# microsoft/Spartan2

Measured on AMD Instinct MI355X. Metric: sha256_spartan prove(): R1CS constraints/sec (prove wall-clock in ms_per_step), higher is better.
Workload: dtype u256 modular integer (8 x u32 Montgomery limbs; T256 scalar/base fields)

## Files before the change

### spartan2_amd/csrc/capi_core.hip

```cpp
#include <atomic>
#include <chrono>
#include <cstdlib>
#include <cstdio>
#include <cstring>

#include "core.hpp"
#include "walk_pool.hpp"
#include "kernels_poly.hpp"
#include "sumcheck_round.hpp"

namespace sp {
static thread_local std::string g_err;
static thread_local sp_wait_hook g_wait_hook = nullptr;
static thread_local void* g_wait_user = nullptr;
void set_error(const std::string& m) { g_err = m; }
static std::atomic<int> g_live_contexts{0};
int live_contexts() { return g_live_contexts.load(std::memory_order_relaxed); }
void relax() {
  if (g_wait_hook) g_wait_hook(g_wait_user);
  else __builtin_ia32_pause();
}
void slow_note(const char* site, long spins) {
  static const bool on = getenv("SPARTAN_SLOWPATH_LOG") != nullptr;
  if (on) fprintf(stderr, "[slow path] %s after %ld polls\n", site, spins);
// ... 1487 lines not shown
      }
      return 1;
    }
    if (round + 1 >= rounds) {
      if (ahead) return 0;
      sp_table* tabs[2] = {A, B};
      have_sums = false;
      int rc2 = launch_bind(c, tabs, 2, rv);
      return rc2 ? rc2 : 1;
    }
    const bool gated = ahead && !launch_ahead_ok(c, A->len);
    if (gated && !gate_ok(c)) return 0;
    if (!stopped && tail_enabled() && A->len <= TAIL_MAX_LEN && table_dense(A) && table_dense(B) && lease.take(tail_blocks(A->len / 2))) {
      spk::TailArgs ta;
      ta.A = A->d;
      ta.B = B->d;
      ta.C = nullptr;
      ta.len = A->len;
      ta.r0 = rv;
      ta.eq_pl = ta.eq_pr = nullptr;
      ta.ell = ta.first_half = ta.rnd0 = 0;
      ta.mail = c->d_mail;
      ta.mirror = c->d_mail_mirror;
      ta.r0_from_mail = ahead ? 1 : 0;
      ta.mapped = c->d_pinned;
      ta.seq0 = next_seq(c);
      ta.hand_n = tail_hand_n(false);
      tail_nb0 = tail_blocks(A->len / 2);
      hipLaunchKernelGGL((spk::k_sumcheck_tail<false>), dim3(tail_nb0), dim3(spk::TAIL_THREADS), 0, c->stream, ta);
      if (!c->tail_ev) (void)hipEventCreateWithFlags(&c->tail_ev, hipEventDisableTiming);
      if (c->tail_ev && hipEventRecord(c->tail_ev, c->stream) == hipSuccess) c->tail_ev_pending = true;
      in_tail = true;
      have_sums = true;
      sp::after_bind(A);
      sp::after_bind(B);
      c->pending_slots = tail_blocks(A->len);
      return 1;
    }
    const bool dense = table_dense(A) && table_dense(B);
    const bool sparse_stream = !dense && A->len / 4 >= STREAM_MIN_Q && sp::eff_lo(A) == A->len / 2 && sp::eff_lo(B) == B->len / 2 && sp::eff_hi(A) <= A->len / 4 && sp::eff_hi(B) <= B->len / 4;
    if (gated && !dense && !sparse_stream) return 0;
    const spk::MailRef mref = gated ? gate_launch(c, answers) : mail_ref(c, ahead, answers);
    if (dense) {
      const size_t q = A->len / 4;
      size_t blocks = (q + chunk - 1) / chunk;
      if (q >= STREAM_MIN_Q) {
        const unsigned seq = next_seq(c);
        const spk::LazyOut lp = lazy_out(c, reinterpret_cast<spk::lazy9_t*>(c->d_scratch), q / 256, 2, nullptr, seq);
        c->timed("bind_stream_quad", 48ull * A->len * 2, [&] {
          hipLaunchKernelGGL(spk::k_bind_eval_quad_stream, dim3((unsigned)(q / 256)), dim3(256), 0, c->stream, A->d, B->d, q, rv, lp, mref);
        });
        sum_lazy_launch(c, lp, q / 256);
      } else {
        c->timed("bind", 48ull * A->len * 2, [&] {
          hipLaunchKernelGGL(spk::k_bind_eval_quad, dim3((unsigned)blocks), dim3(256), 0, c->stream, A->d, B->d, q, rv, c->d_scratch, c->d_pinned, next_seq(c), mref);
        });
        reduce_partials_launch(c, blocks, 2);
      }
      sp::after_bind(A);
      sp::after_bind(B);
      have_sums = true;
      return 1;
    }
    if (sparse_stream) {
      const size_t q = A->len / 4;
      const unsigned seq = next_seq(c);
      const spk::LazyOut lp = lazy_out(c, reinterpret_cast<spk::lazy9_t*>(c->d_scratch), q / 256, 2, nullptr, seq);
      c->timed("bind_stream_quad_sparse", 64ull * (A->len / 2) * 2, [&] {
        hipLaunchKernelGGL(spk::k_bind_eval_quad_stream_sparse, dim3((unsigned)(q / 256)), dim3(256), 0, c->stream, A->d, B->d, q, rv, sp::eff_hi(A), sp::eff_hi(B), lp,
                           mref);
      });
      sum_lazy_launch(c, lp, q / 256);
      sp::after_bind(A);
      sp::after_bind(B);
      have_sums = true;
      return 1;
    }
    if (ahead) return 0;
    sp_table* tabs[2] = {A, B};
    have_sums = false;
    int rc2 = launch_bind(c, tabs, 2, rv);
    return rc2 ? rc2 : 1;
  };
  for (size_t round = 0; round < rounds; ++round) {
    const size_t half = A->len / 2, len_now = A->len;
    const double tr0 = round_trace() ? now_us() : 0;
    fe_t sums[2] = {fe_zero(), fe_zero()};
    bool waiting = have_sums;
    if (!have_sums && !host_mode) {
      size_t len = sp::eff_pairs(A);
      if (sp::eff_pairs(B) < len) len = sp::eff_pairs(B);
      if (half < len) len = half;
      if (len >= STREAM_MIN_Q && len % 1024 == 0) {
        const unsigned seq = next_seq(c);
        const size_t hi_max = sp::eff_hi(A) > sp::eff_hi(B) ? sp::eff_hi(A) : sp::eff_hi(B);
        const bool lowhi = hi_max <= len / 2;
        const size_t blocks = len / (256 * (size_t)4);
        const spk::LazyOut lp = lazy_out(c, reinterpret_cast<spk::lazy9_t*>(c->d_scratch), blocks, 2, nullptr, seq);
        c->timed("eval_quad", 64ull * len + 32ull * ((sp::eff_hi(A) < len ? sp::eff_hi(A) : len) + (sp::eff_hi(B) < len ? sp::eff_hi(B) : len)), [&] {
          if (lowhi)
            hipLaunchKernelGGL((spk::k_eval_quad_stream_lowhi<4>), dim3((unsigned)blocks), dim3(256), 0, c->stream, A->d, B->d, half, sp::eff_hi(A), sp::eff_hi(B), lp);
          else
            hipLaunchKernelGGL((spk::k_eval_quad_stream<4>), dim3((unsigned)blocks), dim3(256), 0, c->stream, A->d, B->d, half, sp::eff_hi(A), sp::eff_hi(B), lp);
        });
        sum_lazy_launch(c, lp, blocks);
        waiting = true;
      } else if (len > 0) {
        size_t blocks = (len + chunk - 1) / chunk;
        c->timed("eval_quad", 64ull * len + 32ull * ((sp::eff_hi(A) < len ? sp::eff_hi(A) : len) + (sp::eff_hi(B) < len ? sp::eff_hi(B) : len)),
                 [&] { hipLaunchKernelGGL(spk::k_eval_quad, dim3((unsigned)blocks), dim3(256), 0, c->stream, A->d, B->d, half, len, sp::eff_hi(A), sp::eff_hi(B), c->d_scratch, c->d_pinned, next_seq(c)); });
        reduce_partials_launch(c, blocks, 2);
        waiting = true;
      }
    }
    const unsigned wait_seq = c->result_seq, wait_slots = c->pending_slots;
    const bool wait_resident = in_tail;
    if (wait_resident && !host_mode && spk::tail_hand_over(len_now, tail_hand_n(false))) {
      hA.resize(2 * len_now);
      if ((rc = wait_hand_over(c, wait_seq, (int)(2 * len_now), hA.data()))) return rc;
      hB = hA.data() + len_now;
      host_mode = true;
      hand_seq = wait_seq;
    }
    if (host_mode) {
      host_quad_eval(hA.data(), hB, half, sums);
      waiting = false;
    }
    if (!host_mode && wait_resident && spk::tail_double(false, len_now, tail_hand_n(false))) {
      fe_t S8[8];
      if ((rc = wait_wide(c, wait_seq, spk::TAIL_DOUBLE_SUMS_QUAD, S8))) return rc;
      if (reduce) {
        int hrc = reduce(reduce_user, reinterpret_cast<uint64_t*>(S8), 8);
        if (hrc) return fail(hrc, "prove_quad: the reduce hook failed");
      }
      fe_t rr[2];
      for (int half2 = 0; half2 < 2; ++half2) {
        fe_t e0, tinf;
        if (half2 == 0) {
          e0 = fe_add<S>(S8[0], S8[1]);
          tinf = fe_add<S>(S8[2], S8[3]);
        } else {
          const fe_t r = rr[0];
          e0 = fe_add<S>(S8[0], fe_mul<S>(r, fe_add<S>(fe_sub<S>(fe_sub<S>(S8[4], S8[0]), S8[2]), fe_mul<S>(r, S8[2]))));
          tinf = fe_add<S>(S8[5], fe_mul<S>(r, fe_add<S>(fe_sub<S>(fe_sub<S>(S8[7], S8[5]), S8[6]), fe_mul<S>(r, S8[6]))));
        }
        UniPoly poly;
        poly.n = 3;
        poly.c[0] = e0;
        poly.c[1] = fe_sub<S>(fe_sub<S>(claim, fe_dbl<S>(e0)), tinf);
        poly.c[2] = tinf;
        absorb_poly(tr->t, poly);
        if (!tr->t.squeeze<S>(lbl_c, 1, &rr[half2])) return fail(SP_ERR_INTERNAL_TRANSCRIPT, "transcript round counter overflow");
        tail_post_challenge(c, rr[half2], wait_seq + half2);
        store_fe(out_r + 4 * (round + half2), rr[half2]);
        store_fe(out_cpolys + 8 * (round + half2), poly.c[0]);
        store_fe(out_cpolys + 8 * (round + half2) + 4, poly.c[2]);
        claim = poly_eval(poly, rr[half2]);
      }
      for (int k = 0; k < 2; ++k) {
        sp::after_bind(A);
        sp::after_bind(B);
        next_seq(c);
      }
      have_sums = round + 2 < rounds;
      c->pending_slots = have_sums ? 1u : 0u;
      last_answered = wait_seq + 1;
      guard.armed = round + 2 < rounds;
      if (observe)
        for (int k = 0; k < 2; ++k) {
          uint64_t rw[4];
          store_fe(rw, rr[k]);
          observe(observe_user, round + k, rw);
        }
      if (round_trace()) fprintf(stderr, "quad rounds %2zu+%2zu len %8zu tail 2 wait+host %7.1f us\n", round, round + 1, len_now, now_us() - tr0);
      ++round;
      continue;
    }
    int issued = 0;
    if (!host_mode && waiting && (in_tail || (c->mail_dev && !reduce))) {
      issued = issue(round, nullptr, wait_seq);
      if (issued < 0) return issued;
      guard.armed = issued != 0;
    }
    if (waiting) {
      const unsigned cur_seq = c->result_seq, cur_slots = c->pending_slots;
      c->result_seq = wait_seq;
      c->pending_slots = wait_slots;
      rc = reduce_partials_wait(c, 2, sums, wait_resident || issued != 0);
      if (issued) {
        c->result_seq = cur_seq;
        c->pending_slots = cur_slots;
      }
      if (rc) return rc;
    }
    if (reduce) {
      int hrc = reduce(reduce_user, reinterpret_cast<uint64_t*>(sums), 2);
      if (hrc) return fail(hrc, "prove_quad: the reduce hook failed");
    }
    const double tr1 = round_trace() ? now_us() : 0;
    fe_t e0 = sums[0], tinf = sums[1];
    UniPoly poly;
    poly.n = 3;
    poly.c[0] = e0;
    poly.c[1] = fe_sub<S>(fe_sub<S>(claim, fe_dbl<S>(e0)), tinf);
    poly.c[2] = tinf;
    absorb_poly(tr->t, poly);
    fe_t r_i;
    if (!tr->t.squeeze<S>(lbl_c, 1, &r_i)) return fail(SP_ERR_INTERNAL_TRANSCRIPT, "transcript round counter overflow");
    last_answered = wait_seq;
    if (host_mode) {
      host_bind_tables(hA.data(), (size_t)(hB - hA.data()), 2, len_now, r_i);
      sp::after_bind(A);
      sp::after_bind(B);
      have_sums = false;
    } else if (issued) {
      tail_post_challenge(c, r_i, wait_seq);
    } else {
      issued = issue(round, &r_i, wait_seq);
      if (issued < 0) return issued;
      if (wait_resident) tail_post_challenge(c, r_i, wait_seq);
    }
    store_fe(out_r + 4 * round, r_i);
    store_fe(out_cpolys + 8 * round, poly.c[0]);
    store_fe(out_cpolys + 8 * round + 4, poly.c[2]);
    claim = poly_eval(poly, r_i);
    guard.armed = in_tail && (host_mode || round + 1 < rounds);
    if (observe) {
      uint64_t rw[4];
      store_fe(rw, r_i);
      observe(observe_user, round, rw);
    }
    if (round_trace()) fprintf(stderr, "quad round %2zu len %8zu tail %d wait %7.1f us host %6.1f us\n", round, len_now, (int)wait_resident, tr1 - tr0, now_us() - tr1);
  }
  if (stopped) {
    store_fe(claim_io, claim);
    return tail_check(c);
  }
  if (host_mode) {
    store_fe(out_final, hA[0]);
    store_fe(out_final + 4, hB[0]);
    tail_post_challenge(c, hA[0], hand_seq);
// ... 1092 lines not shown
```

### spartan2_amd/csrc/kernels_poly.hpp

```cpp
#pragma once
#include "device_utils.hpp"
#include "kernels_shared.hpp"

namespace spk {

constexpr int RESULT_FLAG_ELEM = 7;
__device__ __forceinline__ void publish_result(fe_t* result, unsigned seq) {
  __threadfence_system();
  __hip_atomic_store(reinterpret_cast<unsigned*>(result + RESULT_FLAG_ELEM), seq, __ATOMIC_RELEASE, __HIP_MEMORY_SCOPE_SYSTEM);
}

template <int NACC>
__device__ __forceinline__ void emit_partials_wide(const fe_t (&acc)[NACC], fe_t* __restrict__ mapped, unsigned seq);
template <int NACC>
__device__ __forceinline__ void emit_partials(const fe_t (&acc)[NACC], fe_t* __restrict__ partials, fe_t* __restrict__ mapped, unsigned seq) {
  if (gridDim.x <= HOST_SUM_MAX_BLOCKS) {
    fe_t* slot = mapped + SLOT_BASE_ELEM + 4 * blockIdx.x;
    slot_chk chk = {0u, 0u};
#pragma unroll
    for (int k = 0; k < NACC; ++k) {
      slot_store_elem(slot + k, acc[k]);
      slot_chk_add(chk, acc[k], k);
    }
    slot_store_tag(slot, seq, chk);
// ... 79 lines not shown
    const unsigned* line = mail + MAIL_LINE_WORDS * (want & (MAIL_RING - 1));
    const unsigned* mline = mirror ? mirror + MAIL_LINE_WORDS * (want & (MAIL_RING - 1)) : nullptr;
    const unsigned long long t0 = wall_clock64();
    unsigned long long next_mirror = t0 + MAIL_MIRROR_AFTER_TICKS;
    int good = 0, aborted = 0, from_mirror = 0;
    unsigned w = 0, wdev = 0;
    for (unsigned it = 0;; ++it) {
      if (lane < 13) w = __hip_atomic_load(line + lane, __ATOMIC_RELAXED, __HIP_MEMORY_SCOPE_SYSTEM);
      int st = 0;
      if (__builtin_amdgcn_readlane((int)w, 12) != 0 || ((unsigned)__builtin_amdgcn_readlane((int)w, 8) == want && (unsigned)__builtin_amdgcn_readlane((int)w, 11) == want))
        st = mail_line_state(w, want, lane);
      const bool tick = (it & 15u) == 15u;
      if (st == 0 && mline && tick) {
        const unsigned long long now = wall_clock64();
        if (now >= next_mirror) {
          wdev = w;
          unsigned wm = 0;
          if (lane < 13) wm = __hip_atomic_load(mline + lane, __ATOMIC_RELAXED, __HIP_MEMORY_SCOPE_SYSTEM);
          st = mail_line_state(wm, want, lane);
          if (st != 0) {
            w = wm;
            from_mirror = 1;
          }
          next_mirror = now + MAIL_MIRROR_EVERY_TICKS;
        }
      }
      if (st < 0) {
        aborted = 1;
        break;
      }
      if (st > 0) {
        good = 1;
        break;
      }
      if (tick && wall_clock64() - t0 > MAIL_WATCHDOG_TICKS) break;
    }
    if (lane < 8) r_smem->v[lane] = w;
    if (mline && lane == 0 && (from_mirror || (!good && !aborted))) {
      unsigned* diag = const_cast<unsigned*>(mail) + MAIL_DIAG_WORD;
      if (from_mirror) {
        atomicAdd(diag + 0, 1u);
        diag[2] = want;
      } else {
        atomicAdd(diag + 1, 1u);
      }
    }
    if (mline && from_mirror && lane == 8) const_cast<unsigned*>(mail)[MAIL_DIAG_WORD + 3] = wdev;
    if (!good && !aborted) {
      const unsigned seen = lane < 13 ? w : 0u;
      if (lane < 13) reinterpret_cast<unsigned*>(mapped + TAIL_ERR_ELEM + 1)[lane] = seen;
      if (lane == 0) {
        unsigned* e = reinterpret_cast<unsigned*>(mapped + TAIL_ERR_ELEM);
        e[1] = want;
        e[2] = blockIdx.x;
        e[3] = gridDim.x;
        __hip_atomic_store(e, 1u, __ATOMIC_RELEASE, __HIP_MEMORY_SCOPE_SYSTEM);
      }
    }
    if (lane == 0) ok = good;
  }
  __syncthreads();
  return ok != 0;
}
__device__ __forceinline__ fe_t gated_challenge(const fe_t* p) {
  typedef const __attribute__((address_space(4))) uint32_t* const_words;
  const_words q = (const_words)(uintptr_t)p;
  fe_t r;
#pragma unroll
  for (int i = 0; i < 8; ++i) r.v[i] = q[i];
  return r;
}
__device__ __forceinline__ fe_t challenge_or(const MailRef& m, const fe_t& r_arg) {
  if (m.gated) return gated_challenge(m.gated);
  if (!m.mail) return r_arg;
  __shared__ fe_t r_sh;
  mail_wait(m.mail, m.mirror, m.mapped, m.answers, &r_sh);
  return r_sh;
}

__global__ void __launch_bounds__(64) k_mail_gate(MailRef m, fe_t* __restrict__ out) {
  __shared__ fe_t r_sh;
  mail_wait(m.mail, m.mirror, m.mapped, m.answers, &r_sh);
  if (threadIdx.x < 8) out->v[threadIdx.x] = r_sh.v[threadIdx.x];
}

constexpr int BIND_MAX_TABLES = 8;
struct BindArgs {
  fe_t* z[BIND_MAX_TABLES];
  unsigned long long n[BIND_MAX_TABLES];
  unsigned long long lo[BIND_MAX_TABLES];
  unsigned long long hi[BIND_MAX_TABLES];
  fe_t r;
  fe_t one_minus_r;
};
__global__ void __launch_bounds__(256) k_bind_top(BindArgs a) {
  const int t = blockIdx.y;
  fe_t* __restrict__ Z = a.z[t];
  const unsigned long long n = a.n[t], lo = a.lo[t], hi = a.hi[t];
  const unsigned long long eff = lo > hi ? lo : hi;
  const unsigned long long both = lo < hi ? lo : hi;
  for (unsigned long long i = (unsigned long long)blockIdx.x * blockDim.x + threadIdx.x; i < eff; i += (unsigned long long)gridDim.x * blockDim.x) {
    fe_t out;
    if (i < both) {
      fe_t lo_v = Z[i], hi_v = Z[n + i];
      out = fe_add<S>(lo_v, fe_mul<S>(a.r, fe_sub<S>(hi_v, lo_v)));
    } else if (i < lo) {
      out = fe_mul<S>(Z[i], a.one_minus_r);
    } else {
      out = fe_mul<S>(a.r, Z[n + i]);
    }
    Z[i] = out;
  }
}

__global__ void __launch_bounds__(1024) k_eq_levels(const fe_t* __restrict__ v, int m, fe_t* __restrict__ out) {
  __shared__ fe_t lv[EQ_LDS_ENTRIES];
  eq_levels_block(v + (m - 1), m, out, lv);
}
struct EqPairArgs {
  fe_t v[2][16];
  int m[2];
  fe_t* out[2];
};
__global__ void __launch_bounds__(1024) k_eq_levels_pair(EqPairArgs a) {
  __shared__ fe_t lv[EQ_LDS_ENTRIES];
  const int b = blockIdx.x;
  const int m = a.m[b];
  eq_levels_block(&a.v[b][m - 1], m, a.out[b], lv);
}
constexpr int EQ_LASTK_HPB = 8;
constexpr int EQ_LASTK_BLOCK = 512;
struct EqLastK {
  fe_t w[16];
};
__global__ void __launch_bounds__(EQ_LASTK_BLOCK) k_eq_outer_lastk(const fe_t* __restrict__ t_hi, const fe_t* __restrict__ t_lo, int K, size_t n_hi, EqLastK wk,
                                                                   fe_t* __restrict__ out) {
  constexpr unsigned SLICES = 1024 / EQ_LASTK_BLOCK;
  const unsigned t = threadIdx.x + (blockIdx.x % SLICES) * EQ_LASTK_BLOCK;
  const size_t hi0 = (size_t)(blockIdx.x / SLICES) * EQ_LASTK_HPB;
  fe_t th[EQ_LASTK_HPB];
#pragma unroll
  for (int h = 0; h < EQ_LASTK_HPB; ++h) th[h] = t_hi[hi0 + h < n_hi ? hi0 + h : 0];
  const fe_t lo = fe_mul<S>(t_lo[t >> K], wk.w[t & ((1u << K) - 1)]);
#pragma unroll
  for (int h = 0; h < EQ_LASTK_HPB; ++h) {
    if (hi0 + h >= n_hi) break;
    out[((hi0 + h) << 10) + t] = fe_mul<S>(th[h], lo);
  }
}
__global__ void __launch_bounds__(256) k_eq_outer(const fe_t* __restrict__ t_hi, const fe_t* __restrict__ t_lo, int lo_bits, size_t total,
                                                  fe_t* __restrict__ out) {
  const size_t mask = ((size_t)1 << lo_bits) - 1;
  for (size_t i = (size_t)blockIdx.x * blockDim.x + threadIdx.x; i < total; i += (size_t)gridDim.x * blockDim.x)
    out[i] = fe_mul<S>(t_hi[i >> lo_bits], t_lo[i & mask]);
}

constexpr int EVAL_PPT = 1;
template <int MODE, bool WITH_M1, bool ZC = false>
__global__ void __launch_bounds__(256) k_eval_cubic(const fe_t* __restrict__ A, const fe_t* __restrict__ B, const fe_t* __restrict__ C, size_t half,
                                                    const fe_t* __restrict__ eq_in, const fe_t* __restrict__ eq_out, int s,
                                                    fe_t* __restrict__ partials, fe_t* __restrict__ single_out, unsigned seq) {
  constexpr int NACC = WITH_M1 ? 3 : 2;
  __shared__ fe_t smem[NACC * 4];
  const size_t chunk = (size_t)blockDim.x * EVAL_PPT;
  const size_t base = (size_t)blockIdx.x * chunk;
  const size_t mask = ((size_t)1 << s) - 1;
// ... 243 lines not shown
  bool nz = false;
#pragma unroll
  for (int k = 0; k < PPT; ++k) nz |= !fe_is_zero(p0[k]);
  lazy9_t l0 = lazy_from(fe_zero()), l1 = lazy_from(fe_zero());
#pragma unroll
  for (int k = 0; k < PPT; ++k) l1 = lazy_add(l1, lazy_from(fe_mul<S>(w[k], p1[k])));
  l1 = lazy_wave_sum(l1);
  if (__any(nz)) {
#pragma unroll
    for (int k = 0; k < PPT; ++k) l0 = lazy_add(l0, lazy_from(fe_mul<S>(w[k], p0[k])));
    l0 = lazy_wave_sum(l0);
  }
  stream_block_partials(l0, l1, partials);
}
__global__ void __launch_bounds__(256) k_bind_eval_quad_stream(fe_t* __restrict__ A, fe_t* __restrict__ B, size_t q, fe_t r_arg, LazyOut partials,
                                                               MailRef mref) {
  const size_t id = (size_t)blockIdx.x * blockDim.x + threadIdx.x;
  const fe_t la0 = A[id], la1 = A[id + q], la2 = A[id + 2 * q], la3 = A[id + 3 * q];
  const fe_t lb0 = B[id], lb1 = B[id + q], lb2 = B[id + 2 * q], lb3 = B[id + 3 * q];
  const fe_t r = challenge_or(mref, r_arg);
  const fe_t a0 = bind1(la0, la2, r), a1 = bind1(la1, la3, r);
  const fe_t b0 = bind1(lb0, lb2, r), b1 = bind1(lb1, lb3, r);
  A[id] = a0;
  A[id + q] = a1;
  B[id] = b0;
  B[id + q] = b1;
  stream_block_partials(lazy_wave_sum(lazy_from(fe_mul<S>(a0, b0))), lazy_wave_sum(lazy_from(fe_mul<S>(fe_sub<S>(a1, a0), fe_sub<S>(b1, b0)))), partials);
}
__global__ void __launch_bounds__(256) k_bind_eval_quad_stream_sparse(fe_t* __restrict__ A, fe_t* __restrict__ B, size_t q, fe_t r_arg, size_t hiA, size_t hiB,
                                                                      LazyOut partials, MailRef mref) {
  const size_t id = (size_t)blockIdx.x * blockDim.x + threadIdx.x;
  const fe_t la0 = A[id], la1 = A[id + q], lb0 = B[id], lb1 = B[id + q];
  const fe_t r = challenge_or(mref, r_arg);
  const fe_t one_minus_r = fe_sub<S>(fe_one<S>(), r);
  const fe_t a0 = id < hiA ? bind1(la0, A[id + 2 * q], r) : fe_mul<S>(la0, one_minus_r);
  const fe_t b0 = id < hiB ? bind1(lb0, B[id + 2 * q], r) : fe_mul<S>(lb0, one_minus_r);
  const fe_t a1 = fe_mul<S>(la1, one_minus_r), b1 = fe_mul<S>(lb1, one_minus_r);
  A[id] = a0;
  A[id + q] = a1;
  B[id] = b0;
  B[id + q] = b1;
  stream_block_partials(lazy_wave_sum(lazy_from(fe_mul<S>(a0, b0))), lazy_wave_sum(lazy_from(fe_mul<S>(fe_sub<S>(a1, a0), fe_sub<S>(b1, b0)))), partials);
}
template <int PPT>
__global__ void __launch_bounds__(256) k_eval_quad_stream(const fe_t* __restrict__ A, const fe_t* __restrict__ B, size_t half, size_t hiA, size_t hiB,
                                                          LazyOut partials) {
  const size_t stride = (size_t)gridDim.x * blockDim.x;
  size_t id = (size_t)blockIdx.x * blockDim.x + threadIdx.x;
  lazy9_t l0 = lazy_from(fe_zero()), l1 = lazy_from(fe_zero());
#pragma unroll
  for (int k = 0; k < PPT; ++k, id += stride) {
    const fe_t a0 = A[id], b0 = B[id];
    const fe_t a1 = id < hiA ? A[id + half] : fe_zero(), b1 = id < hiB ? B[id + half] : fe_zero();
    l0 = lazy_add(l0, lazy_from(fe_mul<S>(a0, b0)));
    l1 = lazy_add(l1, lazy_from(fe_mul<S>(fe_sub<S>(a1, a0), fe_sub<S>(b1, b0))));
  }
  stream_block_partials(lazy_wave_sum(l0), lazy_wave_sum(l1), partials);
}
template <int PPT>
__global__ void __launch_bounds__(256) k_eval_quad_stream_lowhi(const fe_t* __restrict__ A, const fe_t* __restrict__ B, size_t half, size_t hiA, size_t hiB,
                                                                LazyOut partials) {
  const size_t stride = (size_t)gridDim.x * blockDim.x;
  const size_t id0 = (size_t)blockIdx.x * blockDim.x + threadIdx.x;
  fe_t a0[PPT], b0[PPT];
#pragma unroll
  for (int k = 0; k < PPT; ++k) {
    a0[k] = A[id0 + k * stride];
    b0[k] = B[id0 + k * stride];
  }
  lazy9_t l0 = lazy_from(fe_zero()), l1 = lazy_from(fe_zero());
#pragma unroll
  for (int k = 0; k < PPT; ++k) {
    const size_t id = id0 + k * stride;
    const fe_t p = fe_mul<S>(a0[k], b0[k]);
    l0 = lazy_add(l0, lazy_from(p));
    if (id < hiA || id < hiB) {
      const fe_t a1 = id < hiA ? A[id + half] : fe_zero(), b1 = id < hiB ? B[id + half] : fe_zero();
      l1 = lazy_add(l1, lazy_from(fe_sub<S>(fe_mul<S>(fe_sub<S>(a1, a0[k]), fe_sub<S>(b1, b0[k])), p)));
    }
  }
  l1 = lazy_add(l1, l0);
  stream_block_partials(lazy_wave_sum(l0), lazy_wave_sum(l1), partials);
}
template <int GL>
__global__ void __launch_bounds__(64) k_sum_partials_lazy(const uint32_t* __restrict__ P, size_t nparts, int gl_rt, const fe_t* __restrict__ eq_out,
                                                          fe_t* __restrict__ mapped, unsigned seq) {
  const int gl = GL >= 0 ? GL : gl_rt;
  const size_t ngroups = nparts >> gl, per = (size_t)1 << gl;
  fe_t acc[2] = {fe_zero(), fe_zero()};
  for (size_t g = (size_t)blockIdx.x * 64 + threadIdx.x; g < ngroups; g += (size_t)gridDim.x * 64) {
    unsigned long long col[2][9];
#pragma unroll
    for (int w = 0; w < 9; ++w)
#pragma unroll
      for (int a = 0; a < 2; ++a) {
        const uint32_t* src = P + (size_t)(2 * w + a) * nparts + g * per;
        if constexpr (GL == 0) {
          col[a][w] = src[0];
        } else if constexpr (GL == 1) {
          const uint2 v = *reinterpret_cast<const uint2*>(src);
          col[a][w] = (unsigned long long)v.x + v.y;
        } else if constexpr (GL == 2) {
          const uint4 v = *reinterpret_cast<const uint4*>(src);
          col[a][w] = ((unsigned long long)v.x + v.y) + ((unsigned long long)v.z + v.w);
        } else if constexpr (GL == 3) {
          const uint4 v = *reinterpret_cast<const uint4*>(src), u = *reinterpret_cast<const uint4*>(src + 4);
          col[a][w] = (((unsigned long long)v.x + v.y) + ((unsigned long long)v.z + v.w)) + (((unsigned long long)u.x + u.y) + ((unsigned long long)u.z + u.w));
        } else {
          unsigned long long t = 0;
          for (size_t k = 0; k < per; ++k) t += src[k];
          col[a][w] = t;
        }
      }
    fe_t f[2];
#pragma unroll
    for (int a = 0; a < 2; ++a) {
      lazy9_t l;
      unsigned long long carry = 0;
#pragma unroll
      for (int w = 0; w < 9; ++w) {
        const unsigned long long t = col[a][w] + carry;
        l.v[w] = (uint32_t)t;
        carry = t >> 32;
      }
      f[a] = lazy_reduce(l);
    }
    if (eq_out) {
      const fe_t eo = eq_out[g];
      f[0] = fe_mul<S>(f[0], eo);
      f[1] = fe_mul<S>(f[1], eo);
    }
    acc[0] = fe_add<S>(acc[0], f[0]);
    acc[1] = fe_add<S>(acc[1], f[1]);
  }
  acc[0] = wave_sum(acc[0]);
  acc[1] = wave_sum(acc[1]);
  if (threadIdx.x == 0) emit_partials<2>(acc, nullptr, mapped, seq);
}

__global__ void __launch_bounds__(256) k_eval_quad(const fe_t* __restrict__ A, const fe_t* __restrict__ B, size_t half, size_t len, size_t hiA, size_t hiB,
                                                   fe_t* __restrict__ partials, fe_t* __restrict__ single_out, unsigned seq) {
  __shared__ fe_t smem[2 * 4];
  const size_t chunk = (size_t)blockDim.x * EVAL_PPT;
  const size_t base = (size_t)blockIdx.x * chunk;
  fe_t acc[2] = {fe_zero(), fe_zero()};
#pragma unroll 1
  for (int k = 0; k < EVAL_PPT; ++k) {
    const size_t id = base + (size_t)k * blockDim.x + threadIdx.x;
    if (id < len) {
      const fe_t a0 = A[id], b0 = B[id];
      const fe_t a1 = id < hiA ? A[id + half] : fe_zero(), b1 = id < hiB ? B[id + half] : fe_zero();
      acc[0] = fe_add<S>(acc[0], fe_mul<S>(a0, b0));
      acc[1] = fe_add<S>(acc[1], fe_mul<S>(fe_sub<S>(a1, a0), fe_sub<S>(b1, b0)));
    }
  }
  block_sum<2>(acc, smem);
  if (threadIdx.x == 0) {
    emit_partials<2>(acc, partials, single_out, seq);
  }
}

template <bool FALLBACK>
__global__ void __launch_bounds__(256) k_eval_cubic_outer_pow(const fe_t* __restrict__ pleft, size_t left, const fe_t* __restrict__ pright, size_t right,
                                                              const fe_t* __restrict__ A, const fe_t* __restrict__ B, const fe_t* __restrict__ C, size_t len,
                                                              fe_t* __restrict__ partials, fe_t* __restrict__ single_out, unsigned seq) {
  __shared__ fe_t smem[3 * 4];
  fe_t acc[3] = {fe_zero(), fe_zero(), fe_zero()};
  const size_t low = (size_t)blockIdx.x * blockDim.x + threadIdx.x;
  if (low < len) {
    fe_t tl, th;
    if (FALLBACK) {
      tl = pleft[low];
      th = pleft[low + len];
    } else {
      const size_t i = low % left, j = low / left;
      const fe_t pl = pleft[i];
      tl = fe_mul<S>(pl, pright[j]);
      th = fe_mul<S>(pl, pright[j + right]);
    }
    const fe_t al = A[low], ah = A[low + len], bl = B[low], bh = B[low + len], cl = C[low], ch = C[low + len];
    acc[0] = fe_mul<S>(tl, fe_sub<S>(fe_mul<S>(al, bl), cl));
    fe_t tb = fe_sub<S>(fe_dbl<S>(th), tl), ab = fe_sub<S>(fe_dbl<S>(ah), al), bb = fe_sub<S>(fe_dbl<S>(bh), bl), cb = fe_sub<S>(fe_dbl<S>(ch), cl);
    acc[1] = fe_mul<S>(tb, fe_sub<S>(fe_mul<S>(ab, bb), cb));
    tb = fe_sub<S>(fe_add<S>(tb, th), tl);
    ab = fe_sub<S>(fe_add<S>(ab, ah), al);
    bb = fe_sub<S>(fe_add<S>(bb, bh), bl);
    cb = fe_sub<S>(fe_add<S>(cb, ch), cl);
    acc[2] = fe_mul<S>(tb, fe_sub<S>(fe_mul<S>(ab, bb), cb));
  }
  block_sum<3>(acc, smem);
  if (threadIdx.x == 0) {
    emit_partials<3>(acc, partials, single_out, seq);
  }
}

struct CubicPairArgs {
  const fe_t *A[2], *B[2], *C[2];
};
template <bool FALLBACK>
__global__ void __launch_bounds__(256) k_eval_cubic_outer_pow_pair(const fe_t* __restrict__ pleft, size_t left, const fe_t* __restrict__ pright, size_t right,
                                                                   CubicPairArgs t, size_t len, unsigned nb, unsigned pp, fe_t* __restrict__ mapped, unsigned seq) {
  __shared__ fe_t smem[3 * 4];
  const unsigned inst = blockIdx.x / nb, bx = blockIdx.x % nb;
  const fe_t* __restrict__ A = t.A[inst];
  const fe_t* __restrict__ B = t.B[inst];
  const fe_t* __restrict__ C = t.C[inst];
  fe_t acc[3] = {fe_zero(), fe_zero(), fe_zero()};
  for (unsigned k = 0; k < pp; ++k) {
    const size_t low = ((size_t)bx * pp + k) * blockDim.x + threadIdx.x;
    if (low >= len) break;
    fe_t tl, th;
    if (FALLBACK) {
      tl = pleft[low];
      th = pleft[low + len];
    } else {
      const size_t i = low % left, j = low / left;
      const fe_t pl = pleft[i];
      tl = fe_mul<S>(pl, pright[j]);
      th = fe_mul<S>(pl, pright[j + right]);
    }
// ... 526 lines not shown
```

Before: 1.024 billion.

## Fuse first two quad sumcheck rounds into one eval and one double-bind pass

Adds a fast path for the first two rounds of the quadratic sumcheck when the high halves of both tables are a short live prefix. One streaming kernel computes the partial sums both rounds need from the quarter tables, plus a small prefix correction. A fused kernel then binds both challenges in one pass, gated on the mailbox so it can be queued ahead. The aim is to avoid one full read/write pass over the tables and one host round trip, at the cost of more complex gating and sums-assembly logic.

After: 1.060 billion (median of 6 runs). +3.5%, better.

```diff
diff --git a/spartan2_amd/csrc/capi_core.hip b/spartan2_amd/csrc/capi_core.hip
--- a/spartan2_amd/csrc/capi_core.hip
+++ b/spartan2_amd/csrc/capi_core.hip
@@ -1593,7 +1593,108 @@
     int rc2 = launch_bind(c, tabs, 2, rv);
     return rc2 ? rc2 : 1;
   };
+  auto two_rounds = [&](const fe_t S8[8], size_t round, unsigned wait_seq, bool post, fe_t rr[2]) -> int {
+    for (int half2 = 0; half2 < 2; ++half2) {
+      fe_t e0, tinf;
+      if (half2 == 0) {
+        e0 = fe_add<S>(S8[0], S8[1]);
+        tinf = fe_add<S>(S8[2], S8[3]);
+      } else {
+        const fe_t r = rr[0];
+        e0 = fe_add<S>(S8[0], fe_mul<S>(r, fe_add<S>(fe_sub<S>(fe_sub<S>(S8[4], S8[0]), S8[2]), fe_mul<S>(r, S8[2]))));
+        tinf = fe_add<S>(S8[5], fe_mul<S>(r, fe_add<S>(fe_sub<S>(fe_sub<S>(S8[7], S8[5]), S8[6]), fe_mul<S>(r, S8[6]))));
+      }
+      UniPoly poly;
+      poly.n = 3;
+      poly.c[0] = e0;
+      poly.c[1] = fe_sub<S>(fe_sub<S>(claim, fe_dbl<S>(e0)), tinf);
+      poly.c[2] = tinf;
+      absorb_poly(tr->t, poly);
+      if (!tr->t.squeeze<S>(lbl_c, 1, &rr[half2])) return fail(SP_ERR_INTERNAL_TRANSCRIPT, "transcript round counter overflow");
+      if (post) tail_post_challenge(c, rr[half2], wait_seq + half2);
+      store_fe(out_r + 4 * (round + half2), rr[half2]);
+      store_fe(out_cpolys + 8 * (round + half2), poly.c[0]);
+      store_fe(out_cpolys + 8 * (round + half2) + 4, poly.c[2]);
+      claim = poly_eval(poly, rr[half2]);
+    }
+    return SP_OK;
+  };
+  static_assert(spk::QUAD2_HI_MAX <= STREAM_MIN_Q, "the two-round kernels take a live prefix of the high halves that lies inside the third quarter");
+  const bool first_two = !reduce && rounds >= 2 && A->len >= 4 * STREAM_MIN_Q && sp::eff_lo(A) == A->len / 2 && sp::eff_lo(B) == B->len / 2 &&
+                         sp::eff_hi(A) <= spk::QUAD2_HI_MAX && sp::eff_hi(B) <= spk::QUAD2_HI_MAX;
+  auto first_two_rounds = [&]() -> int {
+    const double tr0 = round_trace() ? now_us() : 0;
+    const size_t len = A->len, q = len / 4, e = len / 8, hiA = sp::eff_hi(A), hiB = sp::eff_hi(B), hi = hiA > hiB ? hiA : hiB;
+    const unsigned nprefix = (unsigned)((hi + 255) / 256), nparts = (unsigned)(q / 512);
+    spk::lazy9_t* P = reinterpret_cast<spk::lazy9_t*>(c->d_scratch);
+    const unsigned seq = next_seq(c);
+    c->timed("eval_quad", 32ull * len + 128ull * hi + 32ull * (hiA + hiB), [&] {
+      hipLaunchKernelGGL((spk::k_eval_quad2_stream_lowhi<2>), dim3(nprefix + nparts), dim3(256), 0, c->stream, A->d, B->d, q, hiA, hiB, nprefix, P, c->d_pinned, seq);
+    });
+    const unsigned nslots = (unsigned)((nparts / 4 + 63) / 64);
+    hipLaunchKernelGGL((spk::k_sum_partials_lazy<2, 3>), dim3(nslots), dim3(64), 0, c->stream, reinterpret_cast<const uint32_t*>(P), (size_t)nparts, 2,
+                       (const fe_t*)nullptr, c->d_pinned, seq);
+    next_seq(c);
+    const bool more = rounds > 2;
+    auto bind2 = [&](const fe_t* r) {
+      const unsigned seq2 = next_seq(c);
+      const spk::LazyOut lp = lazy_out(c, P, e / 256, 2, nullptr, seq2);
+      fe_t *g0 = nullptr, *g1 = nullptr;
+      if (!r) {
+        g0 = c->d_gate + (seq & (spk::MAIL_RING - 1));
+        g1 = c->d_gate + ((seq + 1) & (spk::MAIL_RING - 1));
+        hipLaunchKernelGGL(spk::k_mail_gate2, dim3(1), dim3(64), 0, c->stream, mail_ref(c, true, seq), g0, g1);
+      }
+      c->timed("bind_stream_quad_sparse", 32ull * len + 32ull * (hiA + hiB) + 64ull * q, [&] {
+        hipLaunchKernelGGL(spk::k_bind2_eval_quad_stream_sparse, dim3((unsigned)(e / 256)), dim3(256), 0, c->stream, A->d, B->d, e, r ? r[0] : fe_zero(),
+                           r ? r[1] : fe_zero(), hiA, hiB, lp, (const fe_t*)g0, (const fe_t*)g1);
+      });
+      if (more) sum_lazy_launch(c, lp, e / 256);
+      else c->pending_slots = 0;
+    };
+    const bool ahead = gate_ok(c);
+    if (ahead) {
+      bind2(nullptr);
+      guard.armed = true;
+    }
+    const unsigned cur_seq = c->result_seq, cur_slots = c->pending_slots;
+    fe_t S3[3], C3[3] = {fe_zero(), fe_zero(), fe_zero()};
+    c->result_seq = seq;
+    c->pending_slots = nslots;
+    int rc2 = reduce_partials_wait(c, 3, S3, ahead);
+    if (!rc2 && nprefix) {
+      c->pending_slots = nprefix;
+      rc2 = reduce_partials_wait(c, 3, C3, ahead, 1, true);
+    }
+    c->result_seq = cur_seq;
+    c->pending_slots = cur_slots;
+    if (rc2) return rc2;
+    const fe_t S8[8] = {S3[0], S3[1], fe_add<S>(S3[0], C3[0]), S3[1], C3[1], S3[2], fe_add<S>(S3[2], C3[2]), C3[1]};
+    fe_t rr[2];
+    if ((rc2 = two_rounds(S8, 0, seq, ahead, rr))) return rc2;
+    guard.armed = false;
+    if (!ahead) bind2(rr);
+    for (int k = 0; k < 2; ++k) {
+      sp::after_bind(A);
+      sp::after_bind(B);
+    }
+    have_sums = more;
+    last_answered = seq + 1;
+    if (observe)
+      for (int k = 0; k < 2; ++k) {
+        uint64_t rw[4];
+        store_fe(rw, rr[k]);
+        observe(observe_user, (size_t)k, rw);
+      }
+    if (round_trace()) fprintf(stderr, "quad rounds %2d+%2d len %8zu tail 0 wait+host %7.1f us\n", 0, 1, len, now_us() - tr0);
+    return SP_OK;
+  };
   for (size_t round = 0; round < rounds; ++round) {
+    if (round == 0 && first_two) {
+      if ((rc = first_two_rounds())) return rc;
+      ++round;
+      continue;
+    }
     const size_t half = A->len / 2, len_now = A->len;
     const double tr0 = round_trace() ? now_us() : 0;
     fe_t sums[2] = {fe_zero(), fe_zero()};
@@ -1645,29 +1746,7 @@
         if (hrc) return fail(hrc, "prove_quad: the reduce hook failed");
       }
       fe_t rr[2];
-      for (int half2 = 0; half2 < 2; ++half2) {
-        fe_t e0, tinf;
-        if (half2 == 0) {
-          e0 = fe_add<S>(S8[0], S8[1]);
-          tinf = fe_add<S>(S8[2], S8[3]);
-        } else {
-          const fe_t r = rr[0];
-          e0 = fe_add<S>(S8[0], fe_mul<S>(r, fe_add<S>(fe_sub<S>(fe_sub<S>(S8[4], S8[0]), S8[2]), fe_mul<S>(r, S8[2]))));
-          tinf = fe_add<S>(S8[5], fe_mul<S>(r, fe_add<S>(fe_sub<S>(fe_sub<S>(S8[7], S8[5]), S8[6]), fe_mul<S>(r, S8[6]))));
-        }
-        UniPoly poly;
-        poly.n = 3;
-        poly.c[0] = e0;
-        poly.c[1] = fe_sub<S>(fe_sub<S>(claim, fe_dbl<S>(e0)), tinf);
-        poly.c[2] = tinf;
-        absorb_poly(tr->t, poly);
-        if (!tr->t.squeeze<S>(lbl_c, 1, &rr[half2])) return fail(SP_ERR_INTERNAL_TRANSCRIPT, "transcript round counter overflow");
-        tail_post_challenge(c, rr[half2], wait_seq + half2);
-        store_fe(out_r + 4 * (round + half2), rr[half2]);
-        store_fe(out_cpolys + 8 * (round + half2), poly.c[0]);
-        store_fe(out_cpolys + 8 * (round + half2) + 4, poly.c[2]);
-        claim = poly_eval(poly, rr[half2]);
-      }
+      if ((rc = two_rounds(S8, round, wait_seq, true, rr))) return rc;
       for (int k = 0; k < 2; ++k) {
         sp::after_bind(A);
         sp::after_bind(B);
diff --git a/spartan2_amd/csrc/kernels_poly.hpp b/spartan2_amd/csrc/kernels_poly.hpp
--- a/spartan2_amd/csrc/kernels_poly.hpp
+++ b/spartan2_amd/csrc/kernels_poly.hpp
@@ -185,6 +185,13 @@
   __shared__ fe_t r_sh;
   mail_wait(m.mail, m.mirror, m.mapped, m.answers, &r_sh);
   if (threadIdx.x < 8) out->v[threadIdx.x] = r_sh.v[threadIdx.x];
+}
+__global__ void __launch_bounds__(64) k_mail_gate2(MailRef m, fe_t* __restrict__ out0, fe_t* __restrict__ out1) {
+  __shared__ fe_t r_sh;
+  const bool ok = mail_wait(m.mail, m.mirror, m.mapped, m.answers, &r_sh);
+  if (threadIdx.x < 8) out0->v[threadIdx.x] = r_sh.v[threadIdx.x];
+  if (ok) mail_wait(m.mail, m.mirror, m.mapped, m.answers + 1, &r_sh);
+  if (threadIdx.x < 8) out1->v[threadIdx.x] = r_sh.v[threadIdx.x];
 }
 
 constexpr int BIND_MAX_TABLES = 8;
@@ -594,19 +601,96 @@
   l1 = lazy_add(l1, l0);
   stream_block_partials(lazy_wave_sum(l0), lazy_wave_sum(l1), partials);
 }
-template <int GL>
+constexpr unsigned long long QUAD2_HI_MAX = 4096;
+__device__ __forceinline__ void stream_block_partials3(const lazy9_t& s0, const lazy9_t& s1, const lazy9_t& s2, lazy9_t* __restrict__ partials, unsigned nparts,
+                                                       unsigned part) {
+  __shared__ lazy9_t sm[4][3];
+  const int lane = threadIdx.x & 63, wave = threadIdx.x >> 6;
+  if (lane == 0) {
+    sm[wave][0] = s0;
+    sm[wave][1] = s1;
+    sm[wave][2] = s2;
+  }
+  __syncthreads();
+  if (threadIdx.x < 3) {
+    const lazy9_t t = lazy_add(lazy_add(sm[0][threadIdx.x], sm[1][threadIdx.x]), lazy_add(sm[2][threadIdx.x], sm[3][threadIdx.x]));
+    uint32_t* P = reinterpret_cast<uint32_t*>(partials);
+#pragma unroll
+    for (int w = 0; w < 9; ++w) P[(size_t)(3 * w + threadIdx.x) * nparts + part] = t.v[w];
+  }
+}
+template <int PPT>
+__global__ void __launch_bounds__(256) k_eval_quad2_stream_lowhi(const fe_t* __restrict__ A, const fe_t* __restrict__ B, size_t q, size_t hiA, size_t hiB,
+                                                                 unsigned nprefix, lazy9_t* __restrict__ partials, fe_t* __restrict__ mapped, unsigned seq) {
+  if (blockIdx.x < nprefix) {
+    __shared__ fe_t smem[3 * 4];
+    const size_t x = (size_t)blockIdx.x * blockDim.x + threadIdx.x;
+    fe_t acc[3] = {fe_zero(), fe_zero(), fe_zero()};
+    if (x < hiA || x < hiB) {
+      const fe_t a0 = A[x], a1 = A[x + q], b0 = B[x], b1 = B[x + q];
+      const fe_t a2 = x < hiA ? A[x + 2 * q] : fe_zero(), b2 = x < hiB ? B[x + 2 * q] : fe_zero();
+      const fe_t u = fe_sub<S>(a1, a0), v = fe_sub<S>(b1, b0);
+      acc[0] = fe_sub<S>(fe_mul<S>(fe_sub<S>(a2, a0), fe_sub<S>(b2, b0)), fe_mul<S>(a0, b0));
+      acc[1] = fe_mul<S>(a2, b2);
+      acc[2] = fe_sub<S>(fe_mul<S>(fe_add<S>(a2, u), fe_add<S>(b2, v)), fe_mul<S>(u, v));
+    }
+    block_sum<3>(acc, smem);
+    if (threadIdx.x == 0) emit_partials_wide<3>(acc, mapped, seq);
+    return;
+  }
+  const unsigned part = blockIdx.x - nprefix, nparts = gridDim.x - nprefix;
+  const size_t stride = (size_t)nparts * blockDim.x;
+  const size_t x0 = (size_t)part * blockDim.x + threadIdx.x;
+  fe_t a0[PPT], a1[PPT], b0[PPT], b1[PPT];
+#pragma unroll
+  for (int k = 0; k < PPT; ++k) {
+    a0[k] = A[x0 + k * stride];
+    a1[k] = A[x0 + k * stride + q];
+    b0[k] = B[x0 + k * stride];
+    b1[k] = B[x0 + k * stride + q];
+  }
+  lazy9_t l0 = lazy_from(fe_zero()), l1 = lazy_from(fe_zero()), l5 = lazy_from(fe_zero());
+#pragma unroll
+  for (int k = 0; k < PPT; ++k) {
+    l0 = lazy_add(l0, lazy_from(fe_mul<S>(a0[k], b0[k])));
+    l1 = lazy_add(l1, lazy_from(fe_mul<S>(a1[k], b1[k])));
+    l5 = lazy_add(l5, lazy_from(fe_mul<S>(fe_sub<S>(a1[k], a0[k]), fe_sub<S>(b1[k], b0[k]))));
+  }
+  stream_block_partials3(lazy_wave_sum(l0), lazy_wave_sum(l1), lazy_wave_sum(l5), partials, nparts, part);
+}
+__global__ void __launch_bounds__(256) k_bind2_eval_quad_stream_sparse(fe_t* __restrict__ A, fe_t* __restrict__ B, size_t e, fe_t r0_arg, fe_t r1_arg, size_t hiA,
+                                                                       size_t hiB, LazyOut partials, const fe_t* __restrict__ g0, const fe_t* __restrict__ g1) {
+  const size_t y = (size_t)blockIdx.x * blockDim.x + threadIdx.x, q = 2 * e;
+  const fe_t la0 = A[y], la0e = A[y + e], la1 = A[y + q], la1e = A[y + q + e];
+  const fe_t lb0 = B[y], lb0e = B[y + e], lb1 = B[y + q], lb1e = B[y + q + e];
+  const fe_t r0 = g0 ? gated_challenge(g0) : r0_arg, r1 = g1 ? gated_challenge(g1) : r1_arg;
+  const fe_t one_minus_r0 = fe_sub<S>(fe_one<S>(), r0);
+  auto bound = [&](const fe_t* __restrict__ T, size_t x, size_t hi, const fe_t& t0, const fe_t& t1) {
+    return x < hi ? bind1(bind1(t0, T[x + 2 * q], r0), fe_mul<S>(t1, one_minus_r0), r1) : fe_mul<S>(bind1(t0, t1, r1), one_minus_r0);
+  };
+  const fe_t a = bound(A, y, hiA, la0, la1), ae = bound(A, y + e, hiA, la0e, la1e);
+  const fe_t b = bound(B, y, hiB, lb0, lb1), be = bound(B, y + e, hiB, lb0e, lb1e);
+  A[y] = a;
+  A[y + e] = ae;
+  B[y] = b;
+  B[y + e] = be;
+  stream_block_partials(lazy_wave_sum(lazy_from(fe_mul<S>(a, b))), lazy_wave_sum(lazy_from(fe_mul<S>(fe_sub<S>(ae, a), fe_sub<S>(be, b)))), partials);
+}
+template <int GL, int NACC = 2>
 __global__ void __launch_bounds__(64) k_sum_partials_lazy(const uint32_t* __restrict__ P, size_t nparts, int gl_rt, const fe_t* __restrict__ eq_out,
                                                           fe_t* __restrict__ mapped, unsigned seq) {
   const int gl = GL >= 0 ? GL : gl_rt;
   const size_t ngroups = nparts >> gl, per = (size_t)1 << gl;
-  fe_t acc[2] = {fe_zero(), fe_zero()};
+  fe_t acc[NACC];
+#pragma unroll
+  for (int a = 0; a < NACC; ++a) acc[a] = fe_zero();
   for (size_t g = (size_t)blockIdx.x * 64 + threadIdx.x; g < ngroups; g += (size_t)gridDim.x * 64) {
-    unsigned long long col[2][9];
+    unsigned long long col[NACC][9];
 #pragma unroll
     for (int w = 0; w < 9; ++w)
 #pragma unroll
-      for (int a = 0; a < 2; ++a) {
-        const uint32_t* src = P + (size_t)(2 * w + a) * nparts + g * per;
+      for (int a = 0; a < NACC; ++a) {
+        const uint32_t* src = P + (size_t)(NACC * w + a) * nparts + g * per;
         if constexpr (GL == 0) {
           col[a][w] = src[0];
         } else if constexpr (GL == 1) {
@@ -624,9 +708,9 @@
           col[a][w] = t;
         }
       }
-    fe_t f[2];
-#pragma unroll
-    for (int a = 0; a < 2; ++a) {
+    fe_t f[NACC];
+#pragma unroll
+    for (int a = 0; a < NACC; ++a) {
       lazy9_t l;
       unsigned long long carry = 0;
 #pragma unroll
@@ -639,15 +723,15 @@
     }
     if (eq_out) {
       const fe_t eo = eq_out[g];
-      f[0] = fe_mul<S>(f[0], eo);
-      f[1] = fe_mul<S>(f[1], eo);
-    }
-    acc[0] = fe_add<S>(acc[0], f[0]);
-    acc[1] = fe_add<S>(acc[1], f[1]);
-  }
-  acc[0] = wave_sum(acc[0]);
-  acc[1] = wave_sum(acc[1]);
-  if (threadIdx.x == 0) emit_partials<2>(acc, nullptr, mapped, seq);
+#pragma unroll
+      for (int a = 0; a < NACC; ++a) f[a] = fe_mul<S>(f[a], eo);
+    }
+#pragma unroll
+    for (int a = 0; a < NACC; ++a) acc[a] = fe_add<S>(acc[a], f[a]);
+  }
+#pragma unroll
+  for (int a = 0; a < NACC; ++a) acc[a] = wave_sum(acc[a]);
+  if (threadIdx.x == 0) emit_partials<NACC>(acc, nullptr, mapped, seq);
 }
 
 __global__ void __launch_bounds__(256) k_eval_quad(const fe_t* __restrict__ A, const fe_t* __restrict__ B, size_t half, size_t len, size_t hiA, size_t hiB,
```
